# OpenGVLab/MM-Interleaved

Measured on NVIDIA H100. Metric: interleaved_steps_per_sec, higher is better.
Workload: dtype bf16

## Files before the change

mm-interleaved_b200/csrc/attn_fwd_sm100.cu:

```cuda
#include "attn_common.cuh"

namespace mmfs {

constexpr int kBM = 128, kBN = 64;
constexpr int kAttnThreads = 288;
constexpr int kConsumers = 256;

template <int HD> constexpr int attn_ctas_per_sm() { return HD == 64 ? 2 : 1; }

template <typename T, int HD, bool LSE>
__global__ void __launch_bounds__(kAttnThreads, attn_ctas_per_sm<HD>())
attn_fwd_kernel(const __grid_constant__ CUtensorMap map_q, const __grid_constant__ CUtensorMap map_k,
                const __grid_constant__ CUtensorMap map_v, const AttnParams p, unsigned *__restrict__ sched, int n_work,
                float *__restrict__ lse) {
    constexpr int NBOX = HD / 64;
    constexpr uint32_t QBOX_BYTES = kBM * 128, KBOX_BYTES = kBN * 128;
    constexpr uint32_t Q_BYTES = NBOX * QBOX_BYTES, KV_BYTES = NBOX * KBOX_BYTES;
    extern __shared__ __align__(1024) uint8_t smem_raw[];
    if ((s_addr(smem_raw) & 1023u) != 0u) { asm volatile("trap;"); }
    uint8_t *sQ = smem_raw;
    uint8_t *sK = sQ + Q_BYTES;
    uint8_t *sV = sK + 2 * KV_BYTES;
    uint64_t *bars = reinterpret_cast<uint64_t *>(sV + 2 * KV_BYTES);
    uint64_t *q_full = bars + 0, *q_empty = bars + 1, *k_full = bars + 2 , *k_empty = bars + 4 ,
             *v_full = bars + 6 , *v_empty = bars + 8 , *item_full = bars + 10 , *item_empty = bars + 12 ;
    int *s_item = reinterpret_cast<int *>(bars + 14);

    const int warp = threadIdx.x >> 5, lane = threadIdx.x & 31;
    const int n_q = (p.Tq + kBM - 1) / kBM;
    auto decode = [&](int w, int &h, int &b, int &q0, int &n_tiles) {
        b = w / (n_q * p.H);
        const int r = w - b * (n_q * p.H);
        const int mi = r / p.H;
        h = r - mi * p.H;
        q0 = (p.causal ? n_q - 1 - mi : mi) * kBM;
        int kv_end = p.Tkv;
        if (p.causal) kv_end = min(p.Tkv, p.past + min(q0 + kBM, p.Tq));
        n_tiles = (kv_end + kBN - 1) / kBN;
    };

    if (threadIdx.x == 0) {
        bar_init(q_full, 1);
        bar_init(q_empty, kConsumers);
        for (int i = 0; i < 2; ++i) {
            bar_init(k_full + i, 1); bar_init(v_full + i, 1); bar_init(k_empty + i, kConsumers); bar_init(v_empty + i, kConsumers);
            bar_init(item_full + i, 1); bar_init(item_empty + i, kConsumers);
        }
        asm volatile("fence.mbarrier_init.release.cluster;" ::: "memory");
    }
    __syncthreads();

    if (warp == 8) {
        if (lane == 0) {
            int w = blockIdx.x;
            int g = 0;
            for (int qn = 0;; ++qn) {
                const int slot = qn & 1;
                if (qn >= 2) bar_wait(item_empty + slot, ((qn >> 1) - 1) & 1);
                s_item[slot] = w < n_work ? w : -1;
                bar_arrive(item_full + slot);
                if (w >= n_work) break;
                const int w_next = sched ? (int)gridDim.x + (int)atomicAdd(sched, 1u) : n_work;
                int h, b, q0, n_tiles;
                decode(w, h, b, q0, n_tiles);
                if (qn > 0) bar_wait(q_empty, (qn - 1) & 1);
                bar_expect_tx(q_full, Q_BYTES);
#pragma unroll
                for (int bx = 0; bx < NBOX; ++bx) tma_load_4d(sQ + bx * QBOX_BYTES, &map_q, q_full, bx * 64, h, q0, b);
                for (int j = 0; j < n_tiles; ++j, ++g) {
                    const int s = g & 1;
                    const uint32_t ph = (g >> 1) & 1;
                    bar_wait(k_empty + s, ph ^ 1);
                    bar_expect_tx(k_full + s, KV_BYTES);
#pragma unroll
                    for (int bx = 0; bx < NBOX; ++bx)
                        tma_load_4d(sK + s * KV_BYTES + bx * KBOX_BYTES, &map_k, k_full + s, bx * 64, h, j * kBN, b);
                    bar_wait(v_empty + s, ph ^ 1);
                    bar_expect_tx(v_full + s, KV_BYTES);
#pragma unroll
                    for (int bx = 0; bx < NBOX; ++bx)
                        tma_load_4d(sV + s * KV_BYTES + bx * KBOX_BYTES, &map_v, v_full + s, bx * 64, h, j * kBN, b);
                }
                w = w_next;
            }
        }
        return;
    }

    const int wg = warp >> 2;
    const int quad = lane >> 2, tq = lane & 3;
    const int row_in_tile = wg * 64 + (warp & 3) * 16 + quad;
    const uint32_t q_base = s_addr(sQ) + wg * 64 * 128;
    int g = 0;
    for (int qn = 0;; ++qn) {
        const int slot = qn & 1;
        bar_wait(item_full + slot, (qn >> 1) & 1);
        const int w = s_item[slot];
        bar_arrive(item_empty + slot);
        if (w < 0) break;
        int h, b, q0, n_tiles;
        decode(w, h, b, q0, n_tiles);
        const int r0 = q0 + row_in_tile;
        float m_run[2] = {-INFINITY, -INFINITY}, l_run[2] = {0.f, 0.f};
        float o[HD / 2];
#pragma unroll
        for (int i = 0; i < HD / 2; ++i) o[i] = 0.f;
        bar_wait(q_full, qn & 1);
        if (n_tiles == 0) bar_arrive(q_empty);

        for (int j = 0; j < n_tiles; ++j, ++g) {
            const int s = g & 1;
            const int k0 = j * kBN;
            float sc[kBN / 2];
            bar_wait(k_full + s, (g >> 1) & 1);
            wgmma_fence();
#pragma unroll
            for (int kk = 0; kk < HD / 16; ++kk)
                Wgmma<T>::ss_n64(sc, smem_desc(q_base + (kk >> 2) * QBOX_BYTES + (kk & 3) * 32, 16, 1024),
                                 smem_desc(s_addr(sK) + s * KV_BYTES + (kk >> 2) * KBOX_BYTES + (kk & 3) * 32, 16, 1024), kk > 0);
            wgmma_commit();
            wgmma_wait<0>();
            reg_fence(sc);
            bar_arrive(k_empty + s);
            if (j + 1 == n_tiles) bar_arrive(q_empty);

            const bool need_mask = (k0 + kBN > p.Tkv) || (p.key_mask != nullptr) ||
                                   (p.causal && k0 + kBN - 1 > p.past + q0 + wg * 64);
            if (need_mask) {
#pragma unroll
                for (int jj = 0; jj < kBN / 8; ++jj)
#pragma unroll
                    for (int c = 0; c < 2; ++c) {
                        const int key = k0 + jj * 8 + 2 * tq + c;
                        bool vis = key < p.Tkv;
                        if (vis && p.key_mask != nullptr) vis = p.key_mask[(long)b * p.Tkv + key] != 0;
#pragma unroll
                        for (int i = 0; i < 2; ++i) {
                            const bool ok = vis && (!p.causal || key <= p.past + r0 + 8 * i);
                            if (!ok) sc[jj * 4 + 2 * i + c] = -INFINITY;
                        }
                    }
            }
            float alpha[2], neg_m[2];
#pragma unroll
            for (int i = 0; i < 2; ++i) {
                float mx = -INFINITY;
#pragma unroll
                for (int jj = 0; jj < kBN / 8; ++jj) mx = fmaxf(mx, fmaxf(sc[jj * 4 + 2 * i], sc[jj * 4 + 2 * i + 1]));
                mx = fmaxf(mx, __shfl_xor_sync(0xffffffffu, mx, 1));
                mx = fmaxf(mx, __shfl_xor_sync(0xffffffffu, mx, 2));
                const float m_new = fmaxf(m_run[i], mx);
                alpha[i] = (m_new == -INFINITY) ? 1.f : fast_exp2((m_run[i] - m_new) * p.scale_log2e);
                m_run[i] = m_new;
                neg_m[i] = (m_new == -INFINITY) ? 0.f : -m_new * p.scale_log2e;
            }
            uint32_t pa[kBN / 16][4];
            float ls[2] = {0.f, 0.f};
#pragma unroll
            for (int jj = 0; jj < kBN / 8; ++jj)
#pragma unroll
                for (int i = 0; i < 2; ++i) {
                    const float e0 = fast_exp2(fmaf(sc[jj * 4 + 2 * i], p.scale_log2e, neg_m[i]));
                    const float e1 = fast_exp2(fmaf(sc[jj * 4 + 2 * i + 1], p.scale_log2e, neg_m[i]));
                    ls[i] += e0 + e1;
                    pa[jj >> 1][(jj & 1) * 2 + i] = pack2<T>(e0, e1);
                }
#pragma unroll
            for (int i = 0; i < 2; ++i) l_run[i] = l_run[i] * alpha[i] + ls[i];
#pragma unroll
            for (int jj = 0; jj < HD / 8; ++jj) {
                o[jj * 4 + 0] *= alpha[0]; o[jj * 4 + 1] *= alpha[0];
                o[jj * 4 + 2] *= alpha[1]; o[jj * 4 + 3] *= alpha[1];
            }

            bar_wait(v_full + s, (g >> 1) & 1);
            reg_fence(o);
            wgmma_fence();
#pragma unroll
            for (int kk = 0; kk < kBN / 16; ++kk) {
                const uint64_t dv = smem_desc(s_addr(sV) + s * KV_BYTES + kk * 16 * 128, KBOX_BYTES, 1024);
                if constexpr (HD == 64) Wgmma<T>::rs_n64(o, pa[kk], dv, 1);
                else Wgmma<T>::rs_n128(o, pa[kk], dv, 1);
            }
            wgmma_commit();
            wgmma_wait<0>();
            reg_fence(o);
            bar_arrive(v_empty + s);
        }

        T *out = static_cast<T *>(p.out) + (long)b * p.o_bs + (long)h * HD;
#pragma unroll
        for (int i = 0; i < 2; ++i) {
            float l = l_run[i];
            l += __shfl_xor_sync(0xffffffffu, l, 1);
            l += __shfl_xor_sync(0xffffffffu, l, 2);
            const float inv = (l > 0.f) ? 1.f / l : 0.f;
            const int q = r0 + 8 * i;
            if constexpr (LSE) {
                if (tq == 0 && q < p.Tq)
                    lse[((long)b * p.H + h) * p.Tq + q] =
                        (l > 0.f) ? fmaf(m_run[i], p.scale_log2e, __log2f(l)) * 0.6931471805599453f : INFINITY;
            }
            if (q < p.Tq) {
                T *op = out + (long)q * p.o_ts + 2 * tq;
#pragma unroll
                for (int jj = 0; jj < HD / 8; ++jj)
                    *reinterpret_cast<uint32_t *>(op + jj * 8) = pack2<T>(o[jj * 4 + 2 * i] * inv, o[jj * 4 + 2 * i + 1] * inv);
            }
        }
    }
}

struct MapKey {
    const void *ptr; int dtype, B, T, H, hd, box_rows; long bs, ts;
    bool operator==(const MapKey &o) const {
        return ptr == o.ptr && dtype == o.dtype && B == o.B && T == o.T && H == o.H && hd == o.hd && box_rows == o.box_rows &&
               bs == o.bs && ts == o.ts;
    }
};
constexpr int kMapCache = 32;
static thread_local MapKey g_map_keys[kMapCache];
static thread_local CUtensorMap g_map_vals[kMapCache];
static thread_local int g_map_n = 0, g_map_next = 0;

static int make_map_uncached(CUtensorMap *map, const void *ptr, int dtype, int B, int T, int H, int hd, long bs, long ts, int box_rows);

static int make_map(CUtensorMap *map, const void *ptr, int dtype, int B, int T, int H, int hd, long bs, long ts, int box_rows) {
    const MapKey key{ptr, dtype, B, T, H, hd, box_rows, bs, ts};
    for (int i = 0; i < g_map_n; ++i)
        if (g_map_keys[i] == key) { *map = g_map_vals[i]; return MMFS_OK; }
    const int rc = make_map_uncached(map, ptr, dtype, B, T, H, hd, bs, ts, box_rows);
    if (rc != MMFS_OK) return rc;
    g_map_keys[g_map_next] = key;
    g_map_vals[g_map_next] = *map;
    g_map_next = (g_map_next + 1) % kMapCache;
    if (g_map_n < kMapCache) ++g_map_n;
    return MMFS_OK;
}

static int make_map_uncached(CUtensorMap *map, const void *ptr, int dtype, int B, int T, int H, int hd, long bs, long ts, int box_rows) {
    EncodeTiledFn fn = tensor_map_encoder();
    if (!fn) { set_error("attn: cuTensorMapEncodeTiled is not available from this driver"); return MMFS_ECUDA; }
    const cuuint64_t dims[4] = {(cuuint64_t)hd, (cuuint64_t)H, (cuuint64_t)T, (cuuint64_t)B};
    const cuuint64_t strides[3] = {(cuuint64_t)hd * 2, (cuuint64_t)ts * 2, (cuuint64_t)bs * 2};
    const cuuint32_t box[4] = {64, 1, (cuuint32_t)box_rows, 1};
    const cuuint32_t estr[4] = {1, 1, 1, 1};
    CUresult r = fn(map, dtype == MMFS_BF16 ? CU_TENSOR_MAP_DATA_TYPE_BFLOAT16 : CU_TENSOR_MAP_DATA_TYPE_FLOAT16, 4,
                    const_cast<void *>(ptr), dims, strides, box, estr, CU_TENSOR_MAP_INTERLEAVE_NONE,
                    CU_TENSOR_MAP_SWIZZLE_128B, CU_TENSOR_MAP_L2_PROMOTION_L2_128B, CU_TENSOR_MAP_FLOAT_OOB_FILL_NONE);
    if (r != CUDA_SUCCESS) { set_error("attn: cuTensorMapEncodeTiled failed (%d)", (int)r); return MMFS_ECUDA; }
    return MMFS_OK;
}

template <typename T, int HD, bool LSE>
static int launch_attn(const CUtensorMap &mq, const CUtensorMap &mk, const CUtensorMap &mv, const AttnParams &p,
                       unsigned *work_counter, float *lse, cudaStream_t st) {
    const int n_q = (p.Tq + kBM - 1) / kBM;
    const long n_work = (long)n_q * p.H * p.B;
    if (n_work >= (1L << 30)) { set_error("attn_forward: %ld work items", n_work); return MMFS_EUNSUPPORTED; }
    constexpr size_t smem = (size_t)(HD / 64) * (kBM * 128 + 4 * kBN * 128) + 14 * 8 + 2 * sizeof(int);
    constexpr auto kern = attn_fwd_kernel<T, HD, LSE>;
    const int rc = ensure_dynamic_smem<kern>(smem);
    if (rc != MMFS_OK) return rc;
    const int resident = attn_ctas_per_sm<HD>() * num_sms();
    const bool persistent = n_work > resident;
    if (persistent) MMFS_CUDA(cudaMemsetAsync(work_counter, 0, sizeof(unsigned), st));
    const int grid = persistent ? resident : (int)n_work;
    kern<<<grid, kAttnThreads, smem, st>>>(mq, mk, mv, p, persistent ? work_counter : nullptr, (int)n_work, lse);
    MMFS_CUDA(cudaGetLastError());
    return MMFS_OK;
}

}

using namespace mmfs;

static int attn_forward(const void *q, const void *k, const void *v, void *out, float *lse, const uint8_t *key_mask,
                        int B, int H, int Tq, int Tkv, int hd, long q_bs, long q_ts, long k_bs, long k_ts, long v_bs,
                        long v_ts, long o_bs, long o_ts, float scale, int causal, int past, int dtype, unsigned *work_counter,
                        void *stream) {
    MMFS_CHECK_ARG(B >= 0 && H > 0 && Tq >= 0 && Tkv > 0, "attn_forward: bad shape");
    if (B == 0 || Tq == 0) return MMFS_OK;
    MMFS_CHECK_ARG(q && k && v && out && work_counter, "attn_forward: null pointer argument");
    MMFS_CHECK_ARG((uintptr_t)work_counter % 4 == 0, "attn_forward: work_counter must be 4-byte aligned");
    if (!(hd == 64 || hd == 128) || !(dtype == MMFS_BF16 || dtype == MMFS_F16)) {
        set_error("attn_forward: tensor-core path needs hd in {64,128} and bf16/f16 (got hd=%d dtype=%d)", hd, dtype);
        return MMFS_EUNSUPPORTED;
    }
    if (((uintptr_t)q | (uintptr_t)k | (uintptr_t)v | (uintptr_t)out) % 16 != 0 ||
        (q_bs | q_ts | k_bs | k_ts | v_bs | v_ts | o_bs | o_ts) % 8 != 0 || B > 65535 || H > 65535) {
        set_error("attn_forward: pointers / strides must be 16-byte aligned; B, H <= 65535");
        return MMFS_EUNSUPPORTED;
    }
    CUtensorMap mq, mk, mv;
    int rc;
    if ((rc = make_map(&mq, q, dtype, B, Tq, H, hd, q_bs, q_ts, kBM)) != MMFS_OK) return rc;
    if ((rc = make_map(&mk, k, dtype, B, Tkv, H, hd, k_bs, k_ts, kBN)) != MMFS_OK) return rc;
    if ((rc = make_map(&mv, v, dtype, B, Tkv, H, hd, v_bs, v_ts, kBN)) != MMFS_OK) return rc;
    AttnParams p;
    p.out = out; p.key_mask = key_mask; p.B = B; p.H = H; p.Tq = Tq; p.Tkv = Tkv; p.causal = causal; p.past = past;
    p.o_bs = o_bs; p.o_ts = o_ts; p.scale_log2e = scale * 1.4426950408889634f;
    cudaStream_t st = (cudaStream_t)stream;
    return dispatch_dtype<kF16Types>(dtype, "attn_forward", [&](auto tag) {
        using T = typename decltype(tag)::type;
        if (lse != nullptr)
            return hd == 64 ? launch_attn<T, 64, true>(mq, mk, mv, p, work_counter, lse, st)
                            : launch_attn<T, 128, true>(mq, mk, mv, p, work_counter, lse, st);
        return hd == 64 ? launch_attn<T, 64, false>(mq, mk, mv, p, work_counter, lse, st)
                        : launch_attn<T, 128, false>(mq, mk, mv, p, work_counter, lse, st);
    });
}

extern "C" int mmfs_attn_forward(const void *q, const void *k, const void *v, void *out, const uint8_t *key_mask,
                                 int B, int H, int Tq, int Tkv, int hd,
                                 long q_bs, long q_ts, long k_bs, long k_ts, long v_bs, long v_ts, long o_bs, long o_ts,
                                 float scale, int causal, int past, int dtype, unsigned *work_counter, void *stream) {
    return attn_forward(q, k, v, out, nullptr, key_mask, B, H, Tq, Tkv, hd, q_bs, q_ts, k_bs, k_ts, v_bs, v_ts, o_bs, o_ts,
                        scale, causal, past, dtype, work_counter, stream);
}

extern "C" int mmfs_attn_forward_lse(const void *q, const void *k, const void *v, void *out, float *lse,
                                     const uint8_t *key_mask, int B, int H, int Tq, int Tkv, int hd,
                                     long q_bs, long q_ts, long k_bs, long k_ts, long v_bs, long v_ts, long o_bs, long o_ts,
                                     float scale, int causal, int past, int dtype, unsigned *work_counter, void *stream) {
    MMFS_CHECK_ARG(lse != nullptr, "attn_forward_lse: null pointer argument (lse)");
    return attn_forward(q, k, v, out, lse, key_mask, B, H, Tq, Tkv, hd, q_bs, q_ts, k_bs, k_ts, v_bs, v_ts, o_bs, o_ts,
                        scale, causal, past, dtype, work_counter, stream);
}
```

mm-interleaved_b200/csrc/tc_common.cuh:

```cuda
#pragma once
#include <cuda.h>

#include "common.cuh"

namespace mmfs {

__device__ __forceinline__ void tma_load_4d(void *dst, const CUtensorMap *map, uint64_t *bar, int c0, int c1, int c2, int c3) {
    asm volatile(
        "cp.async.bulk.tensor.4d.shared::cluster.global.mbarrier::complete_tx::bytes [%0], [%1, {%3, %4, %5, %6}], [%2];" ::
        "r"(s_addr(dst)), "l"(map), "r"(s_addr(bar)), "r"(c0), "r"(c1), "r"(c2), "r"(c3) : "memory");
}
__device__ __forceinline__ void fence_async_smem() { asm volatile("fence.proxy.async.shared::cta;" ::: "memory"); }

__device__ __forceinline__ void wgmma_fence() { asm volatile("wgmma.fence.sync.aligned;" ::: "memory"); }
__device__ __forceinline__ void wgmma_commit() { asm volatile("wgmma.commit_group.sync.aligned;" ::: "memory"); }
template <int N> __device__ __forceinline__ void wgmma_wait() { asm volatile("wgmma.wait_group.sync.aligned %0;" ::"n"(N) : "memory"); }
template <int N> __device__ __forceinline__ void reg_fence(float (&d)[N]) {
#pragma unroll
    for (int i = 0; i < N; ++i) asm volatile("" : "+f"(d[i])::"memory");
}

__device__ __forceinline__ uint64_t smem_desc(uint32_t saddr, uint32_t lbo_bytes, uint32_t sbo_bytes) {
    return (uint64_t)((saddr >> 4) & 0x3fffu) | ((uint64_t)((lbo_bytes >> 4) & 0x3fffu) << 16) |
           ((uint64_t)((sbo_bytes >> 4) & 0x3fffu) << 32) | (1ull << 62);
}

template <typename T> struct Wgmma;
#define MMFS_WGMMA_OPS(TY) \
     \
    __device__ __forceinline__ static void ss_n64(float (&d)[32], uint64_t da, uint64_t db, int acc) { \
        asm volatile( \
            "{\n\t.reg .pred p;\n\tsetp.ne.b32 p, %34, 0;\n\t" \
            "wgmma.mma_async.sync.aligned.m64n64k16.f32." TY "." TY " {%0,%1,%2,%3,%4,%5,%6,%7,%8,%9,%10,%11,%12,%13,%14,%15,%16,%17,%18,%19,%20,%21,%22,%23,%24,%25,%26,%27,%28,%29,%30,%31}, %32, %33, p, 1, 1, 0, 0;\n\t}" \
            : "+f"(d[0]), "+f"(d[1]), "+f"(d[2]), "+f"(d[3]), "+f"(d[4]), "+f"(d[5]), "+f"(d[6]), "+f"(d[7]), "+f"(d[8]), "+f"(d[9]), "+f"(d[10]), "+f"(d[11]), "+f"(d[12]), "+f"(d[13]), "+f"(d[14]), "+f"(d[15]), "+f"(d[16]), "+f"(d[17]), "+f"(d[18]), "+f"(d[19]), "+f"(d[20]), "+f"(d[21]), "+f"(d[22]), "+f"(d[23]), "+f"(d[24]), "+f"(d[25]), "+f"(d[26]), "+f"(d[27]), "+f"(d[28]), "+f"(d[29]), "+f"(d[30]), "+f"(d[31]) \
            : "l"(da), "l"(db), "r"(acc)); \
    } \
     \
    __device__ __forceinline__ static void ss_n128(float (&d)[64], uint64_t da, uint64_t db, int acc) { \
        asm volatile( \
            "{\n\t.reg .pred p;\n\tsetp.ne.b32 p, %66, 0;\n\t" \
            "wgmma.mma_async.sync.aligned.m64n128k16.f32." TY "." TY " {%0,%1,%2,%3,%4,%5,%6,%7,%8,%9,%10,%11,%12,%13,%14,%15,%16,%17,%18,%19,%20,%21,%22,%23,%24,%25,%26,%27,%28,%29,%30,%31,%32,%33,%34,%35,%36,%37,%38,%39,%40,%41,%42,%43,%44,%45,%46,%47,%48,%49,%50,%51,%52,%53,%54,%55,%56,%57,%58,%59,%60,%61,%62,%63}, %64, %65, p, 1, 1, 0, 0;\n\t}" \
            : "+f"(d[0]), "+f"(d[1]), "+f"(d[2]), "+f"(d[3]), "+f"(d[4]), "+f"(d[5]), "+f"(d[6]), "+f"(d[7]), "+f"(d[8]), "+f"(d[9]), "+f"(d[10]), "+f"(d[11]), "+f"(d[12]), "+f"(d[13]), "+f"(d[14]), "+f"(d[15]), "+f"(d[16]), "+f"(d[17]), "+f"(d[18]), "+f"(d[19]), "+f"(d[20]), "+f"(d[21]), "+f"(d[22]), "+f"(d[23]), "+f"(d[24]), "+f"(d[25]), "+f"(d[26]), "+f"(d[27]), "+f"(d[28]), "+f"(d[29]), "+f"(d[30]), "+f"(d[31]), "+f"(d[32]), "+f"(d[33]), "+f"(d[34]), "+f"(d[35]), "+f"(d[36]), "+f"(d[37]), "+f"(d[38]), "+f"(d[39]), "+f"(d[40]), "+f"(d[41]), "+f"(d[42]), "+f"(d[43]), "+f"(d[44]), "+f"(d[45]), "+f"(d[46]), "+f"(d[47]), "+f"(d[48]), "+f"(d[49]), "+f"(d[50]), "+f"(d[51]), "+f"(d[52]), "+f"(d[53]), "+f"(d[54]), "+f"(d[55]), "+f"(d[56]), "+f"(d[57]), "+f"(d[58]), "+f"(d[59]), "+f"(d[60]), "+f"(d[61]), "+f"(d[62]), "+f"(d[63]) \
            : "l"(da), "l"(db), "r"(acc)); \
    } \
     \
    __device__ __forceinline__ static void ss_n160(float (&d)[80], uint64_t da, uint64_t db, int acc) { \
        asm volatile( \
            "{\n\t.reg .pred p;\n\tsetp.ne.b32 p, %82, 0;\n\t" \
            "wgmma.mma_async.sync.aligned.m64n160k16.f32." TY "." TY " {%0,%1,%2,%3,%4,%5,%6,%7,%8,%9,%10,%11,%12,%13,%14,%15,%16,%17,%18,%19,%20,%21,%22,%23,%24,%25,%26,%27,%28,%29,%30,%31,%32,%33,%34,%35,%36,%37,%38,%39,%40,%41,%42,%43,%44,%45,%46,%47,%48,%49,%50,%51,%52,%53,%54,%55,%56,%57,%58,%59,%60,%61,%62,%63,%64,%65,%66,%67,%68,%69,%70,%71,%72,%73,%74,%75,%76,%77,%78,%79}, %80, %81, p, 1, 1, 0, 0;\n\t}" \
            : "+f"(d[0]), "+f"(d[1]), "+f"(d[2]), "+f"(d[3]), "+f"(d[4]), "+f"(d[5]), "+f"(d[6]), "+f"(d[7]), "+f"(d[8]), "+f"(d[9]), "+f"(d[10]), "+f"(d[11]), "+f"(d[12]), "+f"(d[13]), "+f"(d[14]), "+f"(d[15]), "+f"(d[16]), "+f"(d[17]), "+f"(d[18]), "+f"(d[19]), "+f"(d[20]), "+f"(d[21]), "+f"(d[22]), "+f"(d[23]), "+f"(d[24]), "+f"(d[25]), "+f"(d[26]), "+f"(d[27]), "+f"(d[28]), "+f"(d[29]), "+f"(d[30]), "+f"(d[31]), "+f"(d[32]), "+f"(d[33]), "+f"(d[34]), "+f"(d[35]), "+f"(d[36]), "+f"(d[37]), "+f"(d[38]), "+f"(d[39]), "+f"(d[40]), "+f"(d[41]), "+f"(d[42]), "+f"(d[43]), "+f"(d[44]), "+f"(d[45]), "+f"(d[46]), "+f"(d[47]), "+f"(d[48]), "+f"(d[49]), "+f"(d[50]), "+f"(d[51]), "+f"(d[52]), "+f"(d[53]), "+f"(d[54]), "+f"(d[55]), "+f"(d[56]), "+f"(d[57]), "+f"(d[58]), "+f"(d[59]), "+f"(d[60]), "+f"(d[61]), "+f"(d[62]), "+f"(d[63]), "+f"(d[64]), "+f"(d[65]), "+f"(d[66]), "+f"(d[67]), "+f"(d[68]), "+f"(d[69]), "+f"(d[70]), "+f"(d[71]), "+f"(d[72]), "+f"(d[73]), "+f"(d[74]), "+f"(d[75]), "+f"(d[76]), "+f"(d[77]), "+f"(d[78]), "+f"(d[79]) \
            : "l"(da), "l"(db), "r"(acc)); \
    } \
     \
    __device__ __forceinline__ static void rs_n64(float (&d)[32], const uint32_t (&a)[4], uint64_t db, int acc) { \
        asm volatile( \
            "{\n\t.reg .pred p;\n\tsetp.ne.b32 p, %37, 0;\n\t" \
            "wgmma.mma_async.sync.aligned.m64n64k16.f32." TY "." TY " {%0,%1,%2,%3,%4,%5,%6,%7,%8,%9,%10,%11,%12,%13,%14,%15,%16,%17,%18,%19,%20,%21,%22,%23,%24,%25,%26,%27,%28,%29,%30,%31}, {%32,%33,%34,%35}, %36, p, 1, 1, 1;\n\t}" \
            : "+f"(d[0]), "+f"(d[1]), "+f"(d[2]), "+f"(d[3]), "+f"(d[4]), "+f"(d[5]), "+f"(d[6]), "+f"(d[7]), "+f"(d[8]), "+f"(d[9]), "+f"(d[10]), "+f"(d[11]), "+f"(d[12]), "+f"(d[13]), "+f"(d[14]), "+f"(d[15]), "+f"(d[16]), "+f"(d[17]), "+f"(d[18]), "+f"(d[19]), "+f"(d[20]), "+f"(d[21]), "+f"(d[22]), "+f"(d[23]), "+f"(d[24]), "+f"(d[25]), "+f"(d[26]), "+f"(d[27]), "+f"(d[28]), "+f"(d[29]), "+f"(d[30]), "+f"(d[31]) \
            : "r"(a[0]), "r"(a[1]), "r"(a[2]), "r"(a[3]), "l"(db), "r"(acc)); \
    } \
     \
    __device__ __forceinline__ static void rs_n128(float (&d)[64], const uint32_t (&a)[4], uint64_t db, int acc) { \
        asm volatile( \
            "{\n\t.reg .pred p;\n\tsetp.ne.b32 p, %69, 0;\n\t" \
            "wgmma.mma_async.sync.aligned.m64n128k16.f32." TY "." TY " {%0,%1,%2,%3,%4,%5,%6,%7,%8,%9,%10,%11,%12,%13,%14,%15,%16,%17,%18,%19,%20,%21,%22,%23,%24,%25,%26,%27,%28,%29,%30,%31,%32,%33,%34,%35,%36,%37,%38,%39,%40,%41,%42,%43,%44,%45,%46,%47,%48,%49,%50,%51,%52,%53,%54,%55,%56,%57,%58,%59,%60,%61,%62,%63}, {%64,%65,%66,%67}, %68, p, 1, 1, 1;\n\t}" \
            : "+f"(d[0]), "+f"(d[1]), "+f"(d[2]), "+f"(d[3]), "+f"(d[4]), "+f"(d[5]), "+f"(d[6]), "+f"(d[7]), "+f"(d[8]), "+f"(d[9]), "+f"(d[10]), "+f"(d[11]), "+f"(d[12]), "+f"(d[13]), "+f"(d[14]), "+f"(d[15]), "+f"(d[16]), "+f"(d[17]), "+f"(d[18]), "+f"(d[19]), "+f"(d[20]), "+f"(d[21]), "+f"(d[22]), "+f"(d[23]), "+f"(d[24]), "+f"(d[25]), "+f"(d[26]), "+f"(d[27]), "+f"(d[28]), "+f"(d[29]), "+f"(d[30]), "+f"(d[31]), "+f"(d[32]), "+f"(d[33]), "+f"(d[34]), "+f"(d[35]), "+f"(d[36]), "+f"(d[37]), "+f"(d[38]), "+f"(d[39]), "+f"(d[40]), "+f"(d[41]), "+f"(d[42]), "+f"(d[43]), "+f"(d[44]), "+f"(d[45]), "+f"(d[46]), "+f"(d[47]), "+f"(d[48]), "+f"(d[49]), "+f"(d[50]), "+f"(d[51]), "+f"(d[52]), "+f"(d[53]), "+f"(d[54]), "+f"(d[55]), "+f"(d[56]), "+f"(d[57]), "+f"(d[58]), "+f"(d[59]), "+f"(d[60]), "+f"(d[61]), "+f"(d[62]), "+f"(d[63]) \
            : "r"(a[0]), "r"(a[1]), "r"(a[2]), "r"(a[3]), "l"(db), "r"(acc)); \
    }
template <> struct Wgmma<__nv_bfloat16> { MMFS_WGMMA_OPS("bf16") };
template <> struct Wgmma<__half> { MMFS_WGMMA_OPS("f16") };
#undef MMFS_WGMMA_OPS


__device__ __forceinline__ void tma_load_2d(void *dst, const CUtensorMap *map, uint64_t *bar, int c0, int c1) {
    asm volatile(
        "cp.async.bulk.tensor.2d.shared::cluster.global.mbarrier::complete_tx::bytes [%0], [%1, {%3, %4}], [%2];" ::
        "r"(s_addr(dst)), "l"(map), "r"(s_addr(bar)), "r"(c0), "r"(c1) : "memory");
}

typedef CUresult (*EncodeTiledFn)(CUtensorMap *, CUtensorMapDataType, cuuint32_t, void *, const cuuint64_t *, const cuuint64_t *,
                                  const cuuint32_t *, const cuuint32_t *, CUtensorMapInterleave, CUtensorMapSwizzle,
                                  CUtensorMapL2promotion, CUtensorMapFloatOOBfill);

inline EncodeTiledFn tensor_map_encoder() {
    static EncodeTiledFn fn = nullptr;
    if (!fn) {
        void *ptr = nullptr;
        cudaDriverEntryPointQueryResult qres;
        if (cudaGetDriverEntryPoint("cuTensorMapEncodeTiled", &ptr, cudaEnableDefault, &qres) == cudaSuccess &&
            qres == cudaDriverEntryPointSuccess)
            fn = (EncodeTiledFn)ptr;
    }
    return fn;
}

}
```

Measured before the change: 2.673.

## Overlap next-tile QK wgmma with current PV wgmma in hd128 attention forward

Measured after the change: 2.677, median of 6. About the same (+0.1%).

```diff
diff --git a/mm-interleaved_b200/csrc/attn_fwd_sm100.cu b/mm-interleaved_b200/csrc/attn_fwd_sm100.cu
--- a/mm-interleaved_b200/csrc/attn_fwd_sm100.cu
+++ b/mm-interleaved_b200/csrc/attn_fwd_sm100.cu
@@ -108,22 +108,26 @@
         bar_wait(q_full, qn & 1);
         if (n_tiles == 0) bar_arrive(q_empty);
 
-        for (int j = 0; j < n_tiles; ++j, ++g) {
-            const int s = g & 1;
+        float sc[kBN / 2];
+        auto issue_s = [&](int gt) {
+            const int s = gt & 1;
+            bar_wait(k_full + s, (gt >> 1) & 1);
+            uint64_t dq = smem_desc(q_base, 16, 1024), dk = smem_desc(s_addr(sK) + s * KV_BYTES, 16, 1024);
+            asm volatile("" : "+l"(dq), "+l"(dk));
+            wgmma_fence();
+#pragma unroll
+            for (int kk = 0; kk < HD / 16; ++kk)
+                Wgmma<T>::ss_n64(sc, dq + (((kk >> 2) * QBOX_BYTES + (kk & 3) * 32) >> 4),
+                                 dk + (((kk >> 2) * KBOX_BYTES + (kk & 3) * 32) >> 4), kk > 0);
+            wgmma_commit();
+        };
+        auto s_done = [&](int j, int gt) {
+            reg_fence(sc);
+            bar_arrive(k_empty + (gt & 1));
+            if (j + 1 == n_tiles) bar_arrive(q_empty);
+        };
+        auto softmax = [&](int j, uint32_t (&pa)[kBN / 16][4], float (&alpha)[2]) {
             const int k0 = j * kBN;
-            float sc[kBN / 2];
-            bar_wait(k_full + s, (g >> 1) & 1);
-            wgmma_fence();
-#pragma unroll
-            for (int kk = 0; kk < HD / 16; ++kk)
-                Wgmma<T>::ss_n64(sc, smem_desc(q_base + (kk >> 2) * QBOX_BYTES + (kk & 3) * 32, 16, 1024),
-                                 smem_desc(s_addr(sK) + s * KV_BYTES + (kk >> 2) * KBOX_BYTES + (kk & 3) * 32, 16, 1024), kk > 0);
-            wgmma_commit();
-            wgmma_wait<0>();
-            reg_fence(sc);
-            bar_arrive(k_empty + s);
-            if (j + 1 == n_tiles) bar_arrive(q_empty);
-
             const bool need_mask = (k0 + kBN > p.Tkv) || (p.key_mask != nullptr) ||
                                    (p.causal && k0 + kBN - 1 > p.past + q0 + wg * 64);
             if (need_mask) {
@@ -141,7 +145,7 @@
                         }
                     }
             }
-            float alpha[2], neg_m[2];
+            float neg_m[2];
 #pragma unroll
             for (int i = 0; i < 2; ++i) {
                 float mx = -INFINITY;
@@ -154,7 +158,6 @@
                 m_run[i] = m_new;
                 neg_m[i] = (m_new == -INFINITY) ? 0.f : -m_new * p.scale_log2e;
             }
-            uint32_t pa[kBN / 16][4];
             float ls[2] = {0.f, 0.f};
 #pragma unroll
             for (int jj = 0; jj < kBN / 8; ++jj)
@@ -167,13 +170,17 @@
                 }
 #pragma unroll
             for (int i = 0; i < 2; ++i) l_run[i] = l_run[i] * alpha[i] + ls[i];
+        };
+        auto rescale_o = [&](const float (&alpha)[2]) {
 #pragma unroll
             for (int jj = 0; jj < HD / 8; ++jj) {
                 o[jj * 4 + 0] *= alpha[0]; o[jj * 4 + 1] *= alpha[0];
                 o[jj * 4 + 2] *= alpha[1]; o[jj * 4 + 3] *= alpha[1];
             }
-
-            bar_wait(v_full + s, (g >> 1) & 1);
+        };
+        auto issue_pv = [&](const uint32_t (&pa)[kBN / 16][4], int gt) {
+            const int s = gt & 1;
+            bar_wait(v_full + s, (gt >> 1) & 1);
             reg_fence(o);
             wgmma_fence();
 #pragma unroll
@@ -183,9 +190,55 @@
                 else Wgmma<T>::rs_n128(o, pa[kk], dv, 1);
             }
             wgmma_commit();
-            wgmma_wait<0>();
+        };
+        auto pv_done = [&](int gt) {
             reg_fence(o);
-            bar_arrive(v_empty + s);
+            bar_arrive(v_empty + (gt & 1));
+        };
+
+        if constexpr (HD == 128) {
+            if (n_tiles > 0) {
+                uint32_t pa[kBN / 16][4], pb[kBN / 16][4];
+                float alpha[2];
+                issue_s(g);
+                wgmma_wait<0>();
+                s_done(0, g);
+                softmax(0, pa, alpha);
+                rescale_o(alpha);
+                auto tile = [&](int j, uint32_t (&pp)[kBN / 16][4], uint32_t (&pn)[kBN / 16][4]) {
+                    issue_s(g + 1);
+                    issue_pv(pp, g);
+                    wgmma_wait<1>();
+                    s_done(j, g + 1);
+                    softmax(j, pn, alpha);
+                    wgmma_wait<0>();
+                    pv_done(g);
+                    rescale_o(alpha);
+                    ++g;
+                };
+                for (int j = 1;; j += 2) {
+                    if (j >= n_tiles) { issue_pv(pa, g); break; }
+                    tile(j, pa, pb);
+                    if (j + 1 >= n_tiles) { issue_pv(pb, g); break; }
+                    tile(j + 1, pb, pa);
+                }
+                wgmma_wait<0>();
+                pv_done(g);
+                ++g;
+            }
+        } else {
+            for (int j = 0; j < n_tiles; ++j, ++g) {
+                uint32_t pa[kBN / 16][4];
+                float alpha[2];
+                issue_s(g);
+                wgmma_wait<0>();
+                s_done(j, g);
+                softmax(j, pa, alpha);
+                rescale_o(alpha);
+                issue_pv(pa, g);
+                wgmma_wait<0>();
+                pv_done(g);
+            }
         }
 
         T *out = static_cast<T *>(p.out) + (long)b * p.o_bs + (long)h * HD;
```

## Add specialized causal hd128 attention kernel with 128-key tiles and register reallocation

Applied to the files above, without the earlier changes.

New measurement: 2.663 before, 2.682 after, median of 6. About the same (+0.7%).

```diff
diff --git a/mm-interleaved_b200/csrc/attn_fwd_sm100.cu b/mm-interleaved_b200/csrc/attn_fwd_sm100.cu
--- a/mm-interleaved_b200/csrc/attn_fwd_sm100.cu
+++ b/mm-interleaved_b200/csrc/attn_fwd_sm100.cu
@@ -211,6 +211,274 @@
     }
 }
 
+constexpr int kC128Threads = 384;
+constexpr int kC128BN = 128, kC128Stages = 2;
+constexpr int kC128ProducerRegs = 40, kC128ConsumerRegs = 232;
+constexpr int kC128Bars = 2 + 4 * kC128Stages + 4;
+constexpr uint32_t kC128BoxBytes = 128 * 128;
+constexpr uint32_t kC128TileBytes = 2 * kC128BoxBytes;
+constexpr size_t kC128Smem = (size_t)(1 + 2 * kC128Stages) * kC128TileBytes + kC128Bars * 8 + 2 * sizeof(int) +
+                             kConsumers * sizeof(float);
+
+struct RingSlot {
+    int stage;
+    uint32_t parity;
+    __device__ __forceinline__ explicit RingSlot(int g) : stage(g % kC128Stages), parity((uint32_t)(g / kC128Stages) & 1u) {}
+};
+
+template <typename T>
+__global__ void __launch_bounds__(kC128Threads, 1)
+attn_fwd_causal128_kernel(const __grid_constant__ CUtensorMap map_q, const __grid_constant__ CUtensorMap map_k,
+                          const __grid_constant__ CUtensorMap map_v, const AttnParams p, unsigned *__restrict__ sched,
+                          int n_work) {
+    extern __shared__ __align__(1024) uint8_t smem_raw[];
+    if ((s_addr(smem_raw) & 1023u) != 0u) { asm volatile("trap;"); }
+    uint8_t *sQ = smem_raw;
+    uint8_t *sK = sQ + kC128TileBytes;
+    uint8_t *sV = sK + kC128Stages * kC128TileBytes;
+    uint64_t *bars = reinterpret_cast<uint64_t *>(sV + kC128Stages * kC128TileBytes);
+    uint64_t *q_full = bars, *q_empty = bars + 1, *k_full = bars + 2, *k_empty = k_full + kC128Stages,
+             *v_full = k_empty + kC128Stages, *v_empty = v_full + kC128Stages, *item_full = v_empty + kC128Stages,
+             *item_empty = item_full + 2;
+    int *s_item = reinterpret_cast<int *>(bars + kC128Bars);
+    float *s_order = reinterpret_cast<float *>(s_item + 2);
+
+    const int len = p.Tq;
+    const int n_q = (len + kBM - 1) / kBM;
+    auto decode = [&](int w, int &h, int &b, int &q0, int &n_tiles) {
+        b = w / (n_q * p.H);
+        const int r = w - b * (n_q * p.H);
+        const int mi = r / p.H;
+        h = r - mi * p.H;
+        q0 = (n_q - 1 - mi) * kBM;
+        n_tiles = q0 / kC128BN + 1;
+    };
+
+    if (threadIdx.x == 0) {
+        bar_init(q_full, 1);
+        bar_init(q_empty, kConsumers);
+        for (int i = 0; i < kC128Stages; ++i) {
+            bar_init(k_full + i, 1); bar_init(v_full + i, 1); bar_init(k_empty + i, kConsumers); bar_init(v_empty + i, kConsumers);
+        }
+        for (int i = 0; i < 2; ++i) { bar_init(item_full + i, 1); bar_init(item_empty + i, kConsumers); }
+        asm volatile("fence.mbarrier_init.release.cluster;" ::: "memory");
+    }
+    __syncthreads();
+
+    if (threadIdx.x < 128) {
+        setmaxnreg_dec<kC128ProducerRegs>();
+        if (threadIdx.x == 0) {
+            int w = blockIdx.x;
+            int g = 0;
+            for (int qn = 0;; ++qn) {
+                const int slot = qn & 1;
+                if (qn >= 2) bar_wait(item_empty + slot, ((qn >> 1) - 1) & 1);
+                s_item[slot] = w < n_work ? w : -1;
+                bar_arrive(item_full + slot);
+                if (w >= n_work) break;
+                const int w_next = sched ? (int)gridDim.x + (int)atomicAdd(sched, 1u) : n_work;
+                int h, b, q0, n_tiles;
+                decode(w, h, b, q0, n_tiles);
+                if (qn > 0) bar_wait(q_empty, (qn - 1) & 1);
+                bar_expect_tx(q_full, kC128TileBytes);
+                for (int bx = 0; bx < 2; ++bx) tma_load_4d(sQ + bx * kC128BoxBytes, &map_q, q_full, bx * 64, h, q0, b);
+                for (int j = 0; j < n_tiles; ++j, ++g) {
+                    const RingSlot r(g);
+                    bar_wait(k_empty + r.stage, r.parity ^ 1u);
+                    bar_expect_tx(k_full + r.stage, kC128TileBytes);
+                    for (int bx = 0; bx < 2; ++bx)
+                        tma_load_4d(sK + r.stage * kC128TileBytes + bx * kC128BoxBytes, &map_k, k_full + r.stage, bx * 64, h,
+                                    j * kC128BN, b);
+                    bar_wait(v_empty + r.stage, r.parity ^ 1u);
+                    bar_expect_tx(v_full + r.stage, kC128TileBytes);
+                    for (int bx = 0; bx < 2; ++bx)
+                        tma_load_4d(sV + r.stage * kC128TileBytes + bx * kC128BoxBytes, &map_v, v_full + r.stage, bx * 64, h,
+                                    j * kC128BN, b);
+                }
+                w = w_next;
+            }
+        }
+        return;
+    }
+
+    setmaxnreg_inc<kC128ConsumerRegs>();
+    const int wg = (threadIdx.x >> 7) - 1;
+    const int lane = threadIdx.x & 31;
+    const int quad = lane >> 2, tq = lane & 3;
+    const int row_in_tile = wg * 64 + ((threadIdx.x >> 5) & 3) * 16 + quad;
+    const uint32_t q_base = s_addr(sQ) + wg * 64 * 128;
+    const uint32_t order_addr = s_addr(s_order + threadIdx.x - 128);
+
+    auto issue_s = [&](float (&sc)[64], int stage) {
+#pragma unroll
+        for (int kk = 0; kk < 8; ++kk)
+            Wgmma<T>::ss_n128(sc, smem_desc(q_base + (kk >> 2) * kC128BoxBytes + (kk & 3) * 32, 16, 1024),
+                              smem_desc(s_addr(sK) + stage * kC128TileBytes + (kk >> 2) * kC128BoxBytes + (kk & 3) * 32, 16, 1024),
+                              kk > 0);
+    };
+    auto issue_pv = [&](float (&o)[64], const uint32_t (&pa)[4][4], int stage, int hf) {
+#pragma unroll
+        for (int kk = 0; kk < 4; ++kk)
+            Wgmma<T>::rs_n128(o, pa[kk], smem_desc(s_addr(sV) + stage * kC128TileBytes + (4 * hf + kk) * 16 * 128, kC128BoxBytes, 1024), 1);
+    };
+
+    int g = 0;
+    for (int qn = 0;; ++qn) {
+        const int slot = qn & 1;
+        bar_wait(item_full + slot, (qn >> 1) & 1);
+        const int w = s_item[slot];
+        bar_arrive(item_empty + slot);
+        if (w < 0) break;
+        int h, b, q0, n_tiles;
+        decode(w, h, b, q0, n_tiles);
+        const int r0 = q0 + row_in_tile;
+        const int n_half = (min(len, q0 + kBM) + kBN - 1) / kBN;
+        float m_run[2] = {-INFINITY, -INFINITY}, l_run[2] = {0.f, 0.f};
+
+        auto softmax = [&](float (&sc)[64], int j, int hf, float (&alpha)[2]) {
+            const int k0 = j * kC128BN + hf * kBN;
+            float *sh = sc + hf * (kBN / 2);
+            uint32_t kb[2] = {~0u, ~0u};
+            if (p.key_mask != nullptr) {
+                const uint8_t *km = p.key_mask + (long)b * len + k0 + 2 * lane;
+#pragma unroll
+                for (int c = 0; c < 2; ++c) kb[c] = __ballot_sync(0xffffffffu, k0 + 2 * lane + c < len && km[c] != 0);
+            }
+            if ((kb[0] & kb[1]) != ~0u || k0 + kBN > len || k0 + kBN - 1 > q0 + wg * 64) {
+#pragma unroll
+                for (int jj = 0; jj < kBN / 8; ++jj)
+#pragma unroll
+                    for (int c = 0; c < 2; ++c) {
+                        const int key = k0 + jj * 8 + 2 * tq + c;
+                        const bool vis = key < len && ((kb[c] >> (4 * jj + tq)) & 1u);
+#pragma unroll
+                        for (int i = 0; i < 2; ++i)
+                            if (!(vis && key <= r0 + 8 * i)) sh[jj * 4 + 2 * i + c] = -INFINITY;
+                    }
+            }
+            float neg_m[2];
+#pragma unroll
+            for (int i = 0; i < 2; ++i) {
+                float mx = -INFINITY;
+#pragma unroll
+                for (int jj = 0; jj < kBN / 8; ++jj) mx = fmaxf(mx, fmaxf(sh[jj * 4 + 2 * i], sh[jj * 4 + 2 * i + 1]));
+                mx = fmaxf(mx, __shfl_xor_sync(0xffffffffu, mx, 1));
+                mx = fmaxf(mx, __shfl_xor_sync(0xffffffffu, mx, 2));
+                const float m_new = fmaxf(m_run[i], mx);
+                alpha[i] = (m_new == -INFINITY) ? 1.f : fast_exp2((m_run[i] - m_new) * p.scale_log2e);
+                m_run[i] = m_new;
+                neg_m[i] = (m_new == -INFINITY) ? 0.f : -m_new * p.scale_log2e;
+            }
+            float ls[2] = {0.f, 0.f};
+#pragma unroll
+            for (int jj = 0; jj < kBN / 8; ++jj)
+#pragma unroll
+                for (int i = 0; i < 2; ++i) {
+                    const float e0 = fast_exp2(fmaf(sh[jj * 4 + 2 * i], p.scale_log2e, neg_m[i]));
+                    const float e1 = fast_exp2(fmaf(sh[jj * 4 + 2 * i + 1], p.scale_log2e, neg_m[i]));
+                    ls[i] += e0 + e1;
+                    sh[jj * 4 + 2 * i] = e0;
+                    sh[jj * 4 + 2 * i + 1] = e1;
+                }
+#pragma unroll
+            for (int i = 0; i < 2; ++i) l_run[i] = l_run[i] * alpha[i] + ls[i];
+        };
+        auto rescale_and_pack = [&](float (&o)[64], const float (&sc)[64], int hf, const float (&alpha)[2],
+                                    uint32_t (&pa)[4][4]) {
+#pragma unroll
+            for (int jj = 0; jj < 16; ++jj) {
+                o[jj * 4 + 0] *= alpha[0]; o[jj * 4 + 1] *= alpha[0];
+                o[jj * 4 + 2] *= alpha[1]; o[jj * 4 + 3] *= alpha[1];
+            }
+            const float *sh = sc + hf * (kBN / 2);
+#pragma unroll
+            for (int jj = 0; jj < kBN / 8; ++jj)
+#pragma unroll
+                for (int i = 0; i < 2; ++i) pa[jj >> 1][(jj & 1) * 2 + i] = pack2<T>(sh[jj * 4 + 2 * i], sh[jj * 4 + 2 * i + 1]);
+        };
+
+        auto softmax_done = [&]() {
+            asm volatile("st.shared.f32 [%0], %1;" ::"r"(order_addr), "f"(l_run[0] + l_run[1]) : "memory");
+        };
+
+        float o[64], sc[64];
+        uint32_t pa[4][4];
+        float alpha[2];
+#pragma unroll
+        for (int i = 0; i < 64; ++i) o[i] = 0.f;
+        bar_wait(q_full, qn & 1);
+
+        for (int j = 0; j < n_tiles; ++j) {
+            const RingSlot rk(g + j);
+            bar_wait(k_full + rk.stage, rk.parity);
+            wgmma_fence();
+            issue_s(sc, rk.stage);
+            wgmma_commit();
+            if (j > 0) {
+                issue_pv(o, pa, RingSlot(g + j - 1).stage, 1);
+                wgmma_commit();
+                wgmma_wait<1>();
+            } else {
+                wgmma_wait<0>();
+            }
+            reg_fence(sc);
+            bar_arrive(k_empty + rk.stage);
+            if (j + 1 == n_tiles) bar_arrive(q_empty);
+
+            softmax(sc, j, 0, alpha);
+            softmax_done();
+            wgmma_wait<0>();
+            reg_fence(o);
+            reg_fence(pa);
+            if (j > 0) bar_arrive(v_empty + RingSlot(g + j - 1).stage);
+            rescale_and_pack(o, sc, 0, alpha, pa);
+            const RingSlot rv(g + j);
+            bar_wait(v_full + rv.stage, rv.parity);
+            wgmma_fence();
+            issue_pv(o, pa, rv.stage, 0);
+            wgmma_commit();
+
+            if (2 * j + 1 < n_half) {
+                softmax(sc, j, 1, alpha);
+                softmax_done();
+                wgmma_wait<0>();
+                reg_fence(o);
+                reg_fence(pa);
+                rescale_and_pack(o, sc, 1, alpha, pa);
+            }
+        }
+        {
+            const RingSlot rv(g + n_tiles - 1);
+            if (2 * n_tiles == n_half) {
+                wgmma_fence();
+                issue_pv(o, pa, rv.stage, 1);
+                wgmma_commit();
+            }
+            wgmma_wait<0>();
+            reg_fence(o);
+            reg_fence(pa);
+            bar_arrive(v_empty + rv.stage);
+        }
+        g += n_tiles;
+
+        T *out = static_cast<T *>(p.out) + (long)b * p.o_bs + (long)h * 128;
+#pragma unroll
+        for (int i = 0; i < 2; ++i) {
+            float l = l_run[i];
+            l += __shfl_xor_sync(0xffffffffu, l, 1);
+            l += __shfl_xor_sync(0xffffffffu, l, 2);
+            const float inv = (l > 0.f) ? 1.f / l : 0.f;
+            const int q = r0 + 8 * i;
+            if (q < len) {
+                T *op = out + (long)q * p.o_ts + 2 * tq;
+#pragma unroll
+                for (int jj = 0; jj < 16; ++jj)
+                    *reinterpret_cast<uint32_t *>(op + jj * 8) = pack2<T>(o[jj * 4 + 2 * i] * inv, o[jj * 4 + 2 * i + 1] * inv);
+            }
+        }
+    }
+}
+
 struct MapKey {
     const void *ptr; int dtype, B, T, H, hd, box_rows; long bs, ts;
     bool operator==(const MapKey &o) const {
@@ -271,6 +539,27 @@
     return MMFS_OK;
 }
 
+template <typename T>
+static int launch_attn_causal128(const CUtensorMap &mq, const CUtensorMap &mk, const CUtensorMap &mv, const AttnParams &p,
+                                 unsigned *work_counter, cudaStream_t st) {
+    const long n_work = (long)((p.Tq + kBM - 1) / kBM) * p.H * p.B;
+    if (n_work >= (1L << 30)) { set_error("attn_forward: %ld work items", n_work); return MMFS_EUNSUPPORTED; }
+    constexpr auto kern = attn_fwd_causal128_kernel<T>;
+    const int rc = ensure_dynamic_smem<kern>(kC128Smem);
+    if (rc != MMFS_OK) return rc;
+    const int resident = num_sms();
+    const bool persistent = n_work > resident;
+    if (persistent) MMFS_CUDA(cudaMemsetAsync(work_counter, 0, sizeof(unsigned), st));
+    const int grid = persistent ? resident : (int)n_work;
+    kern<<<grid, kC128Threads, kC128Smem, st>>>(mq, mk, mv, p, persistent ? work_counter : nullptr, (int)n_work);
+    MMFS_CUDA(cudaGetLastError());
+    return MMFS_OK;
+}
+
+static bool takes_causal128(int hd, int causal, int past, int Tq, int Tkv, bool lse) {
+    return hd == 128 && causal && past == 0 && Tq == Tkv && !lse;
+}
+
 }
 
 using namespace mmfs;
@@ -292,17 +581,20 @@
         set_error("attn_forward: pointers / strides must be 16-byte aligned; B, H <= 65535");
         return MMFS_EUNSUPPORTED;
     }
+    const bool c128 = takes_causal128(hd, causal, past, Tq, Tkv, lse != nullptr);
+    const int key_rows = c128 ? kC128BN : kBN;
     CUtensorMap mq, mk, mv;
     int rc;
     if ((rc = make_map(&mq, q, dtype, B, Tq, H, hd, q_bs, q_ts, kBM)) != MMFS_OK) return rc;
-    if ((rc = make_map(&mk, k, dtype, B, Tkv, H, hd, k_bs, k_ts, kBN)) != MMFS_OK) return rc;
-    if ((rc = make_map(&mv, v, dtype, B, Tkv, H, hd, v_bs, v_ts, kBN)) != MMFS_OK) return rc;
+    if ((rc = make_map(&mk, k, dtype, B, Tkv, H, hd, k_bs, k_ts, key_rows)) != MMFS_OK) return rc;
+    if ((rc = make_map(&mv, v, dtype, B, Tkv, H, hd, v_bs, v_ts, key_rows)) != MMFS_OK) return rc;
     AttnParams p;
     p.out = out; p.key_mask = key_mask; p.B = B; p.H = H; p.Tq = Tq; p.Tkv = Tkv; p.causal = causal; p.past = past;
     p.o_bs = o_bs; p.o_ts = o_ts; p.scale_log2e = scale * 1.4426950408889634f;
     cudaStream_t st = (cudaStream_t)stream;
     return dispatch_dtype<kF16Types>(dtype, "attn_forward", [&](auto tag) {
         using T = typename decltype(tag)::type;
+        if (c128) return launch_attn_causal128<T>(mq, mk, mv, p, work_counter, st);
         if (lse != nullptr)
             return hd == 64 ? launch_attn<T, 64, true>(mq, mk, mv, p, work_counter, lse, st)
                             : launch_attn<T, 128, true>(mq, mk, mv, p, work_counter, lse, st);
diff --git a/mm-interleaved_b200/csrc/tc_common.cuh b/mm-interleaved_b200/csrc/tc_common.cuh
--- a/mm-interleaved_b200/csrc/tc_common.cuh
+++ b/mm-interleaved_b200/csrc/tc_common.cuh
@@ -19,6 +19,14 @@
 #pragma unroll
     for (int i = 0; i < N; ++i) asm volatile("" : "+f"(d[i])::"memory");
 }
+template <int M, int N> __device__ __forceinline__ void reg_fence(uint32_t (&a)[M][N]) {
+#pragma unroll
+    for (int i = 0; i < M; ++i)
+#pragma unroll
+        for (int j = 0; j < N; ++j) asm volatile("" : "+r"(a[i][j])::"memory");
+}
+template <int N> __device__ __forceinline__ void setmaxnreg_dec() { asm volatile("setmaxnreg.dec.sync.aligned.u32 %0;" ::"n"(N)); }
+template <int N> __device__ __forceinline__ void setmaxnreg_inc() { asm volatile("setmaxnreg.inc.sync.aligned.u32 %0;" ::"n"(N)); }
 
 __device__ __forceinline__ uint64_t smem_desc(uint32_t saddr, uint32_t lbo_bytes, uint32_t sbo_bytes) {
     return (uint64_t)((saddr >> 4) & 0x3fffu) | ((uint64_t)((lbo_bytes >> 4) & 0x3fffu) << 16) |
```
